# jltsiren/bwt-merge

Measured on AMD Instinct MI355X. Metric: merged Gbases/sec (input1+input2), bit-exact native BWT; value = inputs and result resident in HBM, host_to_host_value = SURVEY 8(d)'s T (page-locked host to page-locked host), higher is better.
Workload: dtype u64

## Files before the change

bwt-merge_amd/__init__.py:

```python
from . import build as _build
from . import capi
from .capi import (Builder, BwtmError, Context, Group, HostBuffer, Index, Locator, Part, host_index, partition_cuts_host, window_blocks, RankArray, Slice, device_bytes_peak, fold_offsets, merged_records, slice_bounds, slice_bounds_equal, init, interleave,
                   make_default_current, merge, merge_consume, merge_host, merge_host_pipelined, merge_host_streamed, assemble_pieces, upload_begin, RESULT_ON_DEVICE, pool_stats, pool_poison_stats, profile_enable, profile_only, profile_read, profile_reset,
                   ra_buffer_bytes, synchronize, trim, tune)



def build(force=False, verbose=False, experimental=False):
    return _build.build(force=force, verbose=verbose, experimental=experimental)
```

bwt-merge_amd/capi.py:

```python
import ctypes as C
import os

import numpy as np

HERE = os.path.dirname(os.path.abspath(__file__))
LIB_PATH = os.environ.get("BWTM_LIB") or os.path.join(HERE, "libbwtm.so")
SIGMA = 6

u64 = C.c_uint64
p_u8 = C.POINTER(C.c_uint8)
p_u64 = C.POINTER(C.c_uint64)
vp = C.c_void_p



class HostInput(C.Structure):
    _fields_ = [("data", C.c_void_p), ("nbytes", u64), ("sequences", u64), ("bases", u64), ("C", p_u64)]


class HostOutput(C.Structure):
    _fields_ = [("data", C.c_void_p), ("nbytes", u64), ("blocks", u64), ("sequences", u64), ("bases", u64),
                ("C", u64 * (SIGMA + 1)), ("block_end", C.c_void_p), ("cum", C.c_void_p),
                ("sample_width", C.c_int), ("fields", C.c_void_p), ("anchors", C.c_void_p),
                ("ms_upload", C.c_double), ("ms_search", C.c_double), ("ms_interleave", C.c_double),
# ... 1148 lines not shown
        except Exception:
            pass


class PoolInfo(C.Structure):
    _fields_ = [("held_bytes", u64), ("cached_bytes", u64), ("peak_bytes", u64), ("mapped_blocks", u64), ("address_bytes_reserved", u64),
                ("address_space_exhausted", C.c_int), ("hipmalloc_fallbacks", u64)]


def pool_stats():
    info = PoolInfo()
    check(lib().bwtm_pool_stats(C.byref(info)))
    return {k: int(getattr(info, k)) for k, _ in PoolInfo._fields_}


def pool_poison_stats():
    fills, nbytes = u64(0), u64(0)
    check(lib().bwtm_pool_poison_stats(C.byref(fills), C.byref(nbytes)))
    return int(fills.value), int(nbytes.value)


def profile_enable(on=True):
    check(lib().bwtm_profile_enable(1 if on else 0))


def profile_only(name=None):
    check(lib().bwtm_profile_only(name.encode() if name else None))


def profile_reset():
    check(lib().bwtm_profile_reset())


def profile_read():
    cap = 64
    names = (C.c_char_p * cap)()
    ms = (C.c_double * cap)()
    n = (u64 * cap)()
    k = lib().bwtm_profile_read(names, ms, n, cap)
    return {names[i].decode(): (ms[i], int(n[i])) for i in range(min(k, cap))}
```

bwt-merge_amd/csrc/api/context.hip.h:

```cpp
#pragma once


namespace
{

thread_local std::string g_error;

int fail(int code, const char* fmt, ...)
{
  char buf[512];
  va_list ap; va_start(ap, fmt); vsnprintf(buf, sizeof(buf), fmt, ap); va_end(ap);
  g_error = buf;
  return code;
}

inline u64 div_up(u64 a, u64 b) { return (a + b - 1) / b; }

}


struct bwtm_context
{
  int device = -1;
  hipStream_t stream = nullptr;
  hipStream_t copy_stream = nullptr;
  std::recursive_mutex mu;
  bool is_default = false;
  std::atomic<long long> live_handles{0};

  bool profiling = false;
  std::string profile_only;
  bool profile_open = false;
  struct Pending { const char* name; hipEvent_t start, stop; };
  std::vector<Pending> pending;
  std::map<std::string, std::pair<double, uint64_t>> totals;
  std::vector<const char*> order;

  std::multimap<u64, void*> free_blocks;
  u64 cached_bytes = 0, held_bytes = 0, peak_bytes = 0;
  struct VBlock { u64 bytes = 0; std::vector<hipMemGenericAllocationHandle_t> chunks; hipEvent_t released = nullptr; };
  bool vmm = false;
  std::vector<hipMemGenericAllocationHandle_t> free_chunks;
  std::map<void*, VBlock> vblocks;
  u64 device_total = 0;
  u64 va_fallbacks = 0;

  void* stream_stage[4] = {nullptr, nullptr, nullptr, nullptr};
  u64 stream_stage_cap[4] = {0, 0, 0, 0};
  u64* host_scratch = nullptr;
  u64 scan1_tiles = 0, pull_scan1_tiles = 0;
};

namespace
{

struct Tuning
{
  long long search_algo = 0;
  long long frontier_unfused = 0;
  long long l1_cap = 0;
  long long emit_path = 0;
  long long round_emits = 1ll << 33;
  long long emit_budget = 0;
  long long frontier_epoch = 512;
  long long eager_cum_budget = 16ll << 30;
  long long upload_chunk = 256ll << 20;
  long long download_chunk = 128ll << 20;
  long long range_ratio = 8;
#ifdef BWTM_EXPERIMENTAL
  long long search_view = 0;
#endif
  long long frontier_stage_out = 1;
  long long frontier_parts = 0;
  long long part_capacity = 0;
  long long recs_uniform = 0;
  long long recs_window = 0;
  long long stream_samples_query = 0;
  long long stream_upload = 0;
  long long extract_batch = 1ll << 20;
  long long locate_batch = 1ll << 20;
  long long overlap_batch = 1ll << 20;
  long long ingest_verify = 0;
#ifdef BWTM_DIAGNOSTICS
  long long walk_emit = 0;
  long long walk_blocks = 0;
  long long walk_kernel = 0;
  long long walk_ablate = 0;
  long long walk_variant = 0;
  long long scatter_kernel = 0;
  long long overlap_kernel = 0;
#endif
};
Tuning g_tune;

std::mutex g_registry_mu;
std::map<int, bwtm_context*> g_default_ctx;
thread_local bwtm_context* t_bound = nullptr;
thread_local bwtm_context* t_ctx = nullptr;

#define CTX (*t_ctx)

#define HIP_TRY(expr) do { hipError_t e_ = (expr); if(e_ != hipSuccess) { \
  return fail(e_ == hipErrorOutOfMemory ? BWTM_ENOMEM : BWTM_ENODEV, "%s failed: %s (%s:%d)", #expr, hipGetErrorString(e_), __FILE__, __LINE__); } } while(0)

#define TRY(expr) do { int rc_ = (expr); if(rc_ != BWTM_OK) { return rc_; } } while(0)
// ... 111 lines not shown
{
  if(!CTX.profile_open) { return; }
  (void)hipEventRecord(CTX.pending.back().stop, CTX.stream);
}

void profile_collect()
{
  if(CTX.pending.empty()) { return; }
  (void)hipStreamSynchronize(CTX.stream);
  for(auto& p : CTX.pending)
  {
    float ms = 0; (void)hipEventElapsedTime(&ms, p.start, p.stop);
    auto it = CTX.totals.find(p.name);
    if(it == CTX.totals.end()) { CTX.totals[p.name] = std::make_pair((double)ms, (uint64_t)1); CTX.order.push_back(p.name); }
    else { it->second.first += ms; it->second.second += 1; }
    (void)hipEventDestroy(p.start); (void)hipEventDestroy(p.stop);
  }
  CTX.pending.clear();
}

#define LAUNCH_CFG(name, kernel, gridx, gridy, block, lds, ...) do { \
  const unsigned long long gx_ = (unsigned long long)(gridx); \
  if(gx_ * (unsigned long long)(block) >= (1ull << 32)) { return fail(BWTM_EINVAL, "launch of %s: %llu workgroups of %u threads do not fit one grid", name, gx_, (unsigned)(block)); } \
  profile_begin(name); \
  hipLaunchKernelGGL(kernel, dim3((unsigned)gx_, (unsigned)(gridy)), dim3((unsigned)(block)), (unsigned)(lds), CTX.stream, __VA_ARGS__); \
  profile_end(); \
  hipError_t le_ = hipGetLastError(); \
  if(le_ != hipSuccess) { return fail(BWTM_ENODEV, "launch of %s failed: %s", name, hipGetErrorString(le_)); } } while(0)

#define LAUNCH(name, kernel, grid, block, ...) LAUNCH_CFG(name, kernel, grid, 1, block, 0, __VA_ARGS__)
#define LAUNCH_LDS(name, kernel, grid, block, lds, ...) LAUNCH_CFG(name, kernel, grid, 1, block, lds, __VA_ARGS__)
#define LAUNCH2D(name, kernel, gridx, gridy, block, ...) LAUNCH_CFG(name, kernel, gridx, gridy, block, 0, __VA_ARGS__)
#define LAUNCH_STEP(name, EMIT, HI, VIEW, PULL, grid, ...) do { \
  if(g_tune.frontier_stage_out) { LAUNCH(name, (k_frontier_step<EMIT, HI, VIEW, PULL, true>), grid, FR_BLOCK, __VA_ARGS__); } \
  else { LAUNCH(name, (k_frontier_step<EMIT, HI, VIEW, PULL, false>), grid, FR_BLOCK, __VA_ARGS__); } } while(0)


u64 VMM_CHUNK = 1024ull << 20;
u64 VMM_MIN = 512ull << 20;

u64 pool_round(u64 n)
{
  if(n < 256) { n = 256; }
  u64 g = (n >= (64ull << 20) ? (2ull << 20) : (n >= (1ull << 20) ? (64ull << 10) : 256ull));
  return (n + g - 1) / g * g;
}

bool trace_enabled()
{
  static const bool on = (std::getenv("BWTM_TRACE") != nullptr);
  return on;
}

double trace_now()
{
  return std::chrono::duration<double, std::milli>(std::chrono::steady_clock::now().time_since_epoch()).count();
}

struct AddressSpace
{
  std::mutex mu;
  char* segment = nullptr; u64 segment_size = 0, used = 0;
  u64 reserved_total = 0;
  bool exhausted = false;
};
AddressSpace g_va;
u64 VA_SEGMENT = 8ull << 40, VA_LIMIT = 64ull << 40;

// ... 296 lines not shown

extern "C" void bwtm_context_destroy(bwtm_context* context)
{
  if(!context || context->is_default) { return; }
  if(t_bound == context) { t_bound = nullptr; }
  if(context->live_handles.load() > 0)
  {
    fail(BWTM_EINVAL, "bwtm_context_destroy: %lld handles of the context are still alive; context not destroyed", context->live_handles.load());
    return;
  }
  context_teardown(context);
  delete context;
}

extern "C" const char* bwtm_last_error(void) { return g_error.c_str(); }

namespace
{
int tune_set(const char* key, long long value)
{
  std::string k(key);
  if(k == "search_algo") { g_tune.search_algo = value; }
  else if(k == "frontier_unfused") { g_tune.frontier_unfused = value; }
  else if(k == "l1_cap") { g_tune.l1_cap = value; }
  else if(k == "emit_path") { g_tune.emit_path = value; }
  else if(k == "round_emits") { g_tune.round_emits = (value > 0 ? value : 1); }
  else if(k == "emit_budget") { g_tune.emit_budget = (value > 0 ? value : 0); }
  else if(k == "frontier_epoch") { g_tune.frontier_epoch = (value > 0 ? value : 512); }
  else if(k == "range_ratio") { g_tune.range_ratio = (value >= 0 ? value : 8); }
#ifdef BWTM_EXPERIMENTAL
  else if(k == "search_view") { g_tune.search_view = (value >= 0 && value <= 2 ? value : 0); }
#endif
  else if(k == "frontier_stage_out") { g_tune.frontier_stage_out = (value != 0); }
  else if(k == "frontier_parts") { g_tune.frontier_parts = (value > 0 ? value : 0); }
  else if(k == "stream_samples_query") { g_tune.stream_samples_query = (value != 0); }
  else if(k == "stream_upload") { g_tune.stream_upload = (value != 0); }
  else if(k == "ingest_verify") { g_tune.ingest_verify = (value != 0); }
  else if(k == "extract_batch") { g_tune.extract_batch = (value > 0 ? value : (1ll << 20)); }
  else if(k == "locate_batch") { g_tune.locate_batch = (value > 0 ? std::min<long long>(value, 1ll << 28) : (1ll << 20)); }
  else if(k == "overlap_batch") { g_tune.overlap_batch = (value > 0 ? std::min<long long>(value, 1ll << 28) : (1ll << 20)); }
  else if(k == "part_capacity") { g_tune.part_capacity = value; }
  else if(k == "recs_uniform") { g_tune.recs_uniform = (value > 0 ? 1 : (value < 0 ? -1 : 0)); }
  else if(k == "recs_window") { g_tune.recs_window = (value == 8192 || value == 16384 || value == 32768 ? value : 0); }
  else if(k == "eager_cum_budget") { g_tune.eager_cum_budget = (value > 0 ? value : (16ll << 30)); }
  else if(k == "upload_chunk") { g_tune.upload_chunk = (value > 0 ? value : (256ll << 20)); }
  else if(k == "download_chunk") { g_tune.download_chunk = (value > 0 ? value : (128ll << 20)); }
#ifdef BWTM_DIAGNOSTICS
  else if(k == "walk_emit") { g_tune.walk_emit = value; }
  else if(k == "walk_blocks") { g_tune.walk_blocks = value; }
  else if(k == "walk_kernel") { g_tune.walk_kernel = value; }
  else if(k == "walk_ablate") { g_tune.walk_ablate = value; }
  else if(k == "walk_variant") { g_tune.walk_variant = value; }
  else if(k == "scatter_kernel") { g_tune.scatter_kernel = value; }
  else if(k == "overlap_kernel") { g_tune.overlap_kernel = (value == 1 ? 1 : 0); }
#endif
  else { return fail(BWTM_EINVAL, "bwtm_tune: unknown key %s", key); }
  return BWTM_OK;
}

void apply_env_tuning()
{
  static std::mutex mu;
  static bool done = false;
  std::lock_guard<std::mutex> lock(mu);
  if(done) { return; }
  done = true;
// ... 73 lines not shown
  if(!out) { return fail(BWTM_EINVAL, "bwtm_host_alloc: null argument"); }
  hipError_t e = hipHostMalloc(out, nbytes > 0 ? nbytes : 8, hipHostMallocDefault);
  if(e != hipSuccess) { (void)hipGetLastError(); return fail(BWTM_ENOMEM, "hipHostMalloc(%llu bytes) failed: %s", (unsigned long long)nbytes, hipGetErrorString(e)); }
  return BWTM_OK;
}

extern "C" void bwtm_host_free(void* p)
{
  if(p) { (void)hipHostFree(p); }
}


extern "C" int bwtm_profile_enable(int on)
{
  ENTER(nullptr);
  profile_collect();
  CTX.profiling = (on != 0);
  return BWTM_OK;
}

extern "C" int bwtm_profile_only(const char* name)
{
  ENTER(nullptr);
  profile_collect();
  CTX.profile_only = (name && name[0] ? std::string(",") + name + "," : std::string());
  return BWTM_OK;
}

extern "C" int bwtm_profile_reset(void)
{
  ENTER(nullptr);
  profile_collect();
  CTX.totals.clear(); CTX.order.clear();
  return BWTM_OK;
}

extern "C" int bwtm_profile_read(const char** names, double* total_ms, uint64_t* launches, int capacity)
{
  Scope scope_(nullptr);
  if(scope_.rc != BWTM_OK) { return 0; }
  profile_collect();
  int k = 0;
  for(const char* name : CTX.order)
  {
    if(k < capacity)
    {
      auto& t = CTX.totals[name];
      names[k] = name; total_ms[k] = t.first; launches[k] = t.second;
    }
    k++;
  }
  return k;
}
```

bwt-merge_amd/csrc/api/search.hip.h:

```cpp
#pragma once

struct bwtm_ra
{
  bwtm_context* ctx = nullptr;
  bwtm_ra() : ctx(t_ctx) { if(ctx) { ctx->live_handles++; } }
  ~bwtm_ra() { if(ctx) { ctx->live_handles--; } }
  bwtm_ra(const bwtm_ra&) = delete; bwtm_ra& operator=(const bwtm_ra&) = delete;
  u64 na = 0, nb = 0, n_out = 0;
  u64 nrecs_out = 0, nchunks = 0;
  DevBuf owned_bits;
  void* bits_ptr = nullptr;
  template<class T> T* bits_as() const { return (T*)bits_ptr; }
  DevBuf chunk_base;
  bool finalized = false;
  u64 values = 0;
  bool ranged = false;
  u64 range_first = 0, range_last = 0;
  DevBuf range_rel;
  DevBuf super_boff;
  bool windowed = false;
  u64 win_word_first = 0, win_words = 0;
};

#define WHOLE_RA(ra, who) if((ra)->windowed) { return fail(BWTM_EINVAL, who ": a window of a rank array (bwtm_ra_create_range) only serves the merge over partitioned records and the output-range entry points"); }
// ... 260 lines not shown
  {
    const u64 limit = std::max<u64>(1, std::min<u64>(count / (u64)g_tune.range_ratio, 1ull << 24));
    TRY(range_phase(a, b, seq_first, count, ra, limit, levels));
    if(levels.N == 0) { return BWTM_OK; }
    TRY(range_alive(levels, node_offsets));
    count = levels.alive;
    if(count == 0) { return BWTM_OK; }
  }
  const u64 ntiles = div_up(ra->n_out + 1, 1ull << TILE_SHIFT);
  const u64 nb_max = div_up(count, FR_BLOCK);
  const u64 nseg = 5 * nb_max;
  const u64 fcap = nb_max * FR_BLOCK;

  const u64 per_seq = b->n / (b->m > 0 ? b->m : 1) + 1;
  u64 emit_budget = (u64)g_tune.emit_budget;
  if(emit_budget == 0)
  {
    emit_budget = 16ull << 30;
    size_t free_b = 0, total_b = 0;
    if(hipMemGetInfo(&free_b, &total_b) == hipSuccess) { emit_budget = std::min<u64>(std::max<u64>(emit_budget, ((u64)free_b + CTX.cached_bytes) / 2), 64ull << 30); }
    else { (void)hipGetLastError(); }
  }
  u64 emit_cap = emit_budget / sizeof(unsigned short);
  if(emit_cap > b->n + 64) { emit_cap = b->n + 64; }
  if(emit_cap > 2 * count * per_seq + (1ull << 20)) { emit_cap = 2 * count * per_seq + (1ull << 20); }
  if(emit_cap < count) { emit_cap = count; }
  u64 EPOCH = std::max<u64>(1, (u64)g_tune.frontier_epoch);
  if(g_tune.l1_cap > 0) { emit_cap = (u64)g_tune.l1_cap; }
  else { EPOCH = std::max<u64>(1, std::min<u64>(EPOCH, emit_cap / std::max<u64>(count, 1))); }
  const u64 bound_budget = 2ull << 30;
  if(EPOCH * (ntiles + 1) * sizeof(u32) > bound_budget) { EPOCH = std::max<u64>(1, bound_budget / ((ntiles + 1) * sizeof(u32))); }

  const bool wide = (a->n >= (1ull << 32) || b->n >= (1ull << 32));
  DevBuf lo[2], hi[2], seg_len[2], seg_phys[2], seg_prefix, emit16, emit_base, bound;
  for(int k = 0; k < 2; k++)
  {
    TRY(lo[k].alloc(fcap * 8)); if(wide) { TRY(hi[k].alloc(fcap * 2)); }
    TRY(seg_len[k].alloc((nseg + 1) * sizeof(u64), true)); TRY(seg_phys[k].alloc((nseg + 1) * sizeof(u64), true));
  }
  TRY(seg_prefix.alloc((nseg + 1) * sizeof(u64)));
  DevBuf first_seg; TRY(first_seg.alloc((nb_max + 1) * sizeof(u32)));
  const u32 LOOK = (count >= (1ull << 24) ? 4 : (count >= (1ull << 20) ? 8 : 32));
  struct Events
  {
    hipEvent_t ev[32]; u32 n = 0;
    ~Events() { for(u32 k = 0; k < n; k++) { (void)hipEventDestroy(ev[k]); } }
  } events;
  for(u32 k = 0; k < LOOK; k++) { HIP_TRY(hipEventCreateWithFlags(&events.ev[k], hipEventDisableTiming)); events.n = k + 1; }
  const u64 scan_tiles = div_up(nseg + 1, (u64)SCAN_TILE);
  DevBuf scan_partial; TRY(scan_partial.alloc(scan_tiles * sizeof(u64), true));
  TRY(emit16.alloc((emit_cap + 16) * sizeof(unsigned short)));
  TRY(emit_base.alloc((EPOCH + 1) * sizeof(u64), true));
  TRY(bound.alloc(EPOCH * (ntiles + 1) * sizeof(u32)));
  HIP_TRY(hipMemsetAsync(bound.p, 0xFF, EPOCH * (ntiles + 1) * sizeof(u32), CTX.stream));

  if(node_phase)
  {
    TRY(range_expand(levels, node_offsets, lo[0].as<uint2>(), hi[0].as<unsigned short>()));
    LAUNCH("frontier_init", k_frontier_init_tables, div_up(nseg + 1, BLOCK_THREADS), BLOCK_THREADS, seg_len[0].as<u64>(), seg_phys[0].as<u64>(), nb_max, count);
    levels.release(); node_offsets.release();
  }
  else
  {
    u64 init_items = (fcap > nseg + 1 ? fcap : nseg + 1);
    LAUNCH("frontier_init", k_frontier_init, div_up(init_items, BLOCK_THREADS), BLOCK_THREADS, lo[0].as<uint2>(), hi[0].as<unsigned short>(),
      seg_len[0].as<u64>(), seg_phys[0].as<u64>(), nb_max, seq_first, count, a->m);
  }
  int cur = 0;
  u64 in_epoch = 0;
  u64 alive_bound = count, epoch_used = 0;
// ... 38 lines not shown
      if(scan_tiles > 1)
      {
        LAUNCH("scan_reduce", k_scan_reduce<0>, scan_tiles, BLOCK_THREADS, seg_len[cur].as<const u64>(), scan_partial.as<u64>(), nseg + 1, (u64)0, scan_tiles);
      }
      LAUNCH("frontier_scan", k_frontier_scan, scan_tiles, BLOCK_THREADS, seg_len[cur].as<const u64>(), scan_partial.as<const u64>(), nseg,
        seg_prefix.as<u64>(), first_seg.as<u32>(), emit_base.as<u64>(), in_epoch, host_ring + (t % LOOK));
      size_in_ring = true;
    }
    else
    {
      TRY(device_scan<0>(seg_len[cur].as<u64>(), seg_prefix.as<u64>(), nseg + 1));
      LAUNCH("frontier_prep", k_frontier_prep, div_up(nseg, BLOCK_THREADS), BLOCK_THREADS, seg_prefix.as<const u64>(), nseg, first_seg.as<u32>(),
        emit_base.as<u64>(), in_epoch);
    }
    if(!size_in_ring) { TRY(fetch_u64(seg_prefix.as<u64>() + nseg, 64 + (u32)(t % LOOK))); HIP_TRY(hipEventRecord(events.ev[t % LOOK], CTX.stream)); }
    {
      const u64 need = std::max<u64>(1, div_up(alive_bound, FR_BLOCK));
      if(g_tune.frontier_parts <= 1 && need * 4 < grid * 3) { grid = need; }
      const int nxt = 1 - cur;
      if(written[nxt] > grid)
      {
        for(u64 c = 0; c < 5; c++) { HIP_TRY(hipMemsetAsync(seg_len[nxt].as<u64>() + c * nb_max + grid, 0, (written[nxt] - grid) * sizeof(u64), CTX.stream)); }
      }
      written[nxt] = grid;
    }
    FrontierView f;
    f.lo = lo[cur].as<const uint2>(); f.hi = hi[cur].as<const unsigned short>();
    f.lo_next = lo[1 - cur].as<uint2>(); f.hi_next = hi[1 - cur].as<unsigned short>();
    f.seg_prefix = seg_prefix.as<const u64>(); f.seg_phys = seg_phys[cur].as<const u64>(); f.first_seg = first_seg.as<const u32>();
    f.seg_len_next = seg_len[1 - cur].as<u64>(); f.seg_phys_next = seg_phys[1 - cur].as<u64>();
    f.nb_max = nb_max;
    f.emit16 = emit16.as<unsigned short>(); f.emit_base = emit_base.as<const u64>(); f.emit_cap = emit_cap; f.bits32 = ra->bits_as<u32>();
    f.bound_row = bound.as<u32>() + in_epoch * (ntiles + 1); f.step = in_epoch; f.block_base = 0; f.src_lo = nullptr; f.src_hi = nullptr; f.nseg_in = 0;
#ifdef BWTM_DIAGNOSTICS
    if(g_tune.walk_emit == 1 && wide) { LAUNCH_STEP("frontier_step_noemit", 1, true, false, false, grid, a->view(), b->view(), f); }
    else if(g_tune.walk_emit == 1) { LAUNCH_STEP("frontier_step_noemit", 1, false, false, false, grid, a->view(), b->view(), f); }
    else
#endif
    if(g_tune.frontier_parts > 1)
    {
      const u64 parts = (u64)g_tune.frontier_parts, per = div_up(nb_max, parts);
      for(u64 part = 0; part < parts && part * per < nb_max; part++)
      {
        f.block_base = (u32)(part * per);
        const u64 nb_part = std::min<u64>(per, nb_max - part * per);
        const char* label = (part == 0 ? "frontier_step_slice0" : "frontier_step_slices");
        if(wide) { LAUNCH_STEP(label, 0, true, false, false, nb_part, a->view(), b->view(), f); }
        else { LAUNCH_STEP(label, 0, false, false, false, nb_part, a->view(), b->view(), f); }
      }
    }
#ifdef BWTM_EXPERIMENTAL
    else if(use_view && wide) { LAUNCH_STEP("frontier_step", 0, true, true, false, grid, a->view(), b->view(), f); }
    else if(use_view) { LAUNCH_STEP("frontier_step", 0, false, true, false, grid, a->view(), b->view(), f); }
#endif
    else if(wide) { LAUNCH_STEP("frontier_step", 0, true, false, false, grid, a->view(), b->view(), f); }
    else { LAUNCH_STEP("frontier_step", 0, false, false, false, grid, a->view(), b->view(), f); }
    if(size_in_ring) { HIP_TRY(hipEventRecord(events.ev[t % LOOK], CTX.stream)); }
    cur = 1 - cur;
    in_epoch++; epoch_used += alive_bound;
    if(in_epoch == EPOCH || (g_tune.l1_cap == 0 && epoch_used + alive_bound > emit_cap))
    {
      TRY(frontier_flush(ra, emit16, emit_cap, emit_base, bound, ntiles, in_epoch));
      HIP_TRY(hipMemsetAsync(bound.p, 0xFF, EPOCH * (ntiles + 1) * sizeof(u32), CTX.stream));
      HIP_TRY(hipMemsetAsync(emit_base.p, 0, (EPOCH + 1) * sizeof(u64), CTX.stream));
      in_epoch = 0; epoch_used = 0;
    }
  }
  TRY(frontier_flush(ra, emit16, emit_cap, emit_base, bound, ntiles, in_epoch));
  return BWTM_OK;
}

}


extern "C" uint64_t bwtm_ra_buffer_bytes(const bwtm_index* a, const bwtm_index* b)
{
  if(!a || !b) { return 0; }
  return div_up(num_records(a->n + b->n), 64) * CHUNK_WORDS * sizeof(u64);
}

extern "C" int bwtm_ra_create_on(const bwtm_index* a, const bwtm_index* b, void* device_buffer, uint64_t nbytes, bwtm_ra** out)
{
  if(!a || !b || !out) { return fail(BWTM_EINVAL, "bwtm_ra_create: null argument"); }
  if(a->ctx != b->ctx) { return fail(BWTM_EINVAL, "bwtm_ra_create: the two indexes live in different contexts"); }
  ENTER(a->ctx);
  bwtm_ra* ra = new bwtm_ra();
  ra->ctx = t_ctx;
  ra->na = a->n; ra->nb = b->n; ra->n_out = a->n + b->n;
  ra->nrecs_out = num_records(ra->n_out);
// ... 168 lines not shown
```

bwt-merge_amd/csrc/kernels/search_frontier.hip.h:

```cpp
#pragma once


constexpr int FR_BLOCK = 256;
constexpr u32 PULL_SRC_SHIFT_ = 56;
constexpr u64 PULL_PHYS_MASK_ = (1ull << PULL_SRC_SHIFT_) - 1;
constexpr int FR_SEGS = 31;

struct FrontierView
{
  const uint2* lo; const unsigned short* hi;
  uint2* lo_next; unsigned short* hi_next;
  const u64* seg_prefix;
  const u64* seg_phys;
  const u32* first_seg;
  u64* seg_len_next; u64* seg_phys_next;
  u64 nb_max;
  unsigned short* emit16;
  const u64* emit_base;
  u64 emit_cap;
  u32* bits32;
  u32* bound_row;
  u64 step;
  u32 block_base;
  const uint2* const* src_lo; const unsigned short* const* src_hi;
// ... 33 lines not shown
__device__ inline void record_words(const RecordFetch& rf, u32 w[16])
{
#pragma unroll
  for(int k = 0; k < 4; k++) { w[4 * k] = rf.v[k].x; w[4 * k + 1] = rf.v[k].y; w[4 * k + 2] = rf.v[k].z; w[4 * k + 3] = rf.v[k].w; }
}

__device__ inline u64 ordinary_lf(const IndexView& X, u64 pos, u32& c, bool want_symbol)
{
  const uint4* p = X.recs + 4 * (pos >> REC_SHIFT);
  const u32 j = (u32)(pos & (REC_POS - 1));
  if(want_symbol)
  {
    const uint4 ch = p[j >> 5];
    const u32 t = j & 31;
    c = ((ch.x >> t) & 1u) | (((ch.y >> t) & 1u) << 1) | (((ch.z >> t) & 1u) << 2);
  }
  if(c == 0) { return 0; }
  u32 total = 0; u32 h[4];
#pragma unroll
  for(u32 k = 0; k < 4; k++)
  {
    const uint4 ch = p[k];
    total += (u32)__builtin_popcount(plane_match(ch.x, ch.y, ch.z, c) & below_mask(j, k));
    h[k] = ch.w;
  }
  const u32 sh = FIELD_BITS * (c - 1);
  const u64 lo = (u64)h[0] | ((u64)h[1] << 32), hi = (u64)h[2] | ((u64)h[3] << 32);
  u64 v;
  if(sh < 64) { v = lo >> sh; if(sh + FIELD_BITS > 64) { v |= hi << (64 - sh); } }
  else { v = hi >> (sh - 64); }
  return X.sup[(pos >> SUPER_SHIFT) * SUP_STRIDE + c] + ((u32)v & FIELD_MASK) + total;
}

template<int EMIT, bool HI, bool VIEW = false, bool PULL = false, bool STAGE = false>
__global__ void __launch_bounds__(FR_BLOCK, (VIEW ? 6 : 8)) k_frontier_step(IndexView A, IndexView B, FrontierView f)
{
  __shared__ u32 wave_cnt[FR_BLOCK / WAVE][6];
  __shared__ uint2 s_out[STAGE ? FR_BLOCK : 1];
  __shared__ unsigned short s_out_hi[STAGE && HI ? FR_BLOCK : 1];
  __shared__ u64 s_prefix[FR_SEGS + 1], s_phys[FR_SEGS + 1];
  __shared__ const uint2* s_src_lo[PULL ? 16 : 1];
  __shared__ const unsigned short* s_src_hi[PULL ? 16 : 1];
  const u64 nseg_out = 5 * f.nb_max;
  const u64 nseg = (PULL ? f.nseg_in : nseg_out);
  const u64 N = f.seg_prefix[nseg];
  const u32 bid = blockIdx.x + f.block_base;
  const u64 g0 = (u64)bid * FR_BLOCK;
  const u32 lane = lane_id(), wave = threadIdx.x >> 6;

  if(g0 >= N)
  {
    if(threadIdx.x < 5) { f.seg_len_next[(u64)threadIdx.x * f.nb_max + bid] = 0; f.seg_phys_next[(u64)threadIdx.x * f.nb_max + bid] = g0; }
    if(bid == 0 && threadIdx.x == 5) { f.seg_len_next[nseg_out] = 0; }
    return;
  }
  const u64 first_seg = f.first_seg[bid];
  if(threadIdx.x <= FR_SEGS)
  {
    u64 sidx = first_seg + threadIdx.x; if(sidx > nseg) { sidx = nseg; }
    s_prefix[threadIdx.x] = f.seg_prefix[sidx];
    s_phys[threadIdx.x] = f.seg_phys[sidx < nseg ? sidx : nseg - 1];
  }
  if(PULL && threadIdx.x >= 64 && threadIdx.x < 80)
  {
    s_src_lo[threadIdx.x - 64] = f.src_lo[threadIdx.x - 64];
    if(HI) { s_src_hi[threadIdx.x - 64] = f.src_hi[threadIdx.x - 64]; }
  }
  __syncthreads();

  const u64 g = g0 + threadIdx.x;
  const bool active = (g < N);
  u64 i = 0, r = 0;
  if(active)
  {
    u64 phys;
    u32 k = 0;
#pragma unroll
    for(u32 step = 16; step != 0; step >>= 1) { if(s_prefix[k + step] <= g) { k += step; } }
    if(k < (u32)FR_SEGS) { phys = s_phys[k] + (g - s_prefix[k]); }
    else
    {
      u64 lo_s = first_seg + FR_SEGS, hi_s = nseg;
      while(hi_s - lo_s > 1)
      {
        const u64 mid = (lo_s + hi_s) >> 1;
        if(f.seg_prefix[mid] <= g) { lo_s = mid; } else { hi_s = mid; }
      }
      const u64 sgm = lo_s;
      phys = f.seg_phys[sgm] + (g - f.seg_prefix[sgm]);
    }
    const uint2* lo_src = f.lo; const unsigned short* hi_src = f.hi;
    if(PULL)
    {
      const u32 src = (u32)(phys >> PULL_SRC_SHIFT_);
      phys &= PULL_PHYS_MASK_;
      lo_src = s_src_lo[src]; if(HI) { hi_src = s_src_hi[src]; }
    }
    uint2 l; u32 h = 0;
    if(PULL) { l = peer_load(&lo_src[phys]); if(HI) { h = (u32)peer_load(&hi_src[phys]); } }
    else { l = lo_src[phys]; if(HI) { h = (u32)hi_src[phys]; } }
    __builtin_amdgcn_sched_barrier(0);
    i = (u64)l.x | ((u64)(h & 0xFF) << 32);
    r = (u64)l.y | ((u64)(h >> 8) << 32);
  }
  const u64 any_active = __ballot(active);
  u32 tile_first = 0xFFFFFFFFu, tile_last = 0xFFFFFFFFu;
  u32 c = 0;
  u64 ni = 0, nr = 0;
  if(any_active != 0)
  {
    const u32 last_lane = 63 - (u32)__builtin_clzll(any_active);
    const u64 li = shfl_u64(i, (int)last_lane), lr = shfl_u64(r, (int)last_lane);
    if(EMIT == 0)
    {
      const u64 p = i + r;
      const u64 my_tile = p >> TILE_SHIFT;
      const u64 prev_tile = shfl_up_u64(my_tile, 1);
      if(active)
      {
        u64 slot = f.emit_base[f.step] + g;
        if(slot < f.emit_cap) { nt_store(&f.emit16[slot], (unsigned short)(p & TILE_MASK)); }
        else { sink_fallback(f.bits32, p); }
        if(lane != 0 && my_tile != prev_tile) { atomicMin(&f.bound_row[my_tile], (u32)g); }
      }
      tile_first = (u32)my_tile;
      tile_last = (u32)shfl_u64(my_tile, (int)last_lane);
    }
#ifdef BWTM_EXPERIMENTAL
    if(VIEW)
    {
      const u64 pi = (active ? i : li), pr = (active ? r : lr);
      const u64 qb = pi / VIEW_POS, qa = pr / VIEW_POS;
      const u32 jb = (u32)(pi - qb * VIEW_POS), ja = (u32)(pr - qa * VIEW_POS);
      RecordFetch fb = record_issue(B.view, B.nview, qb);
      RecordFetch fa = record_issue(A.view, A.nview, qa);
      const u64 vs_b0 = shfl_u64(qb, 0) >> VIEW_SUPER_SHIFT, vs_a0 = shfl_u64(qa, 0) >> VIEW_SUPER_SHIFT;
// ... 41 lines not shown
        ni += cb; nr += ca;
      }
    }
    else
#endif
    {
      u32 wb[16];
      const u64 rec_b = (active ? i : li) >> REC_SHIFT, rec_a = (active ? r : lr) >> REC_SHIFT;
      RecordFetch fb = record_issue(B.recs, B.nrecs, rec_b);
      RecordFetch fa = record_issue(A.recs, A.nrecs, rec_a);
      const u64 sup_b0 = shfl_u64(i, 0) >> SUPER_SHIFT, sup_a0 = shfl_u64(r, 0) >> SUPER_SHIFT;
      const u64* row_b = B.sup + sup_b0 * SUP_STRIDE;
      const u64* row_a = A.sup + sup_a0 * SUP_STRIDE;
      record_words(fb, wb);
      if(active) { c = rec_symbol(wb, (u32)(i & (REC_POS - 1))); }
      u64 supb = 0, supa = 0;
      if(active && c != 0)
      {
        if((i >> SUPER_SHIFT) == sup_b0) { supb = (c == 1 ? row_b[1] : (c == 2 ? row_b[2] : (c == 3 ? row_b[3] : (c == 4 ? row_b[4] : row_b[5])))); }
        else { supb = B.sup[(i >> SUPER_SHIFT) * SUP_STRIDE + c]; }
        if((r >> SUPER_SHIFT) == sup_a0) { supa = (c == 1 ? row_a[1] : (c == 2 ? row_a[2] : (c == 3 ? row_a[3] : (c == 4 ? row_a[4] : row_a[5])))); }
        else { supa = A.sup[(r >> SUPER_SHIFT) * SUP_STRIDE + c]; }
        ni = rec_header(wb, c) + rec_count(wb, c, (u32)(i & (REC_POS - 1)));
      }
      u32 wa[16];
      record_words(fa, wa);
      if(active)
      {
        const u32 ja = (u32)(r & (REC_POS - 1));
        if(c != 0)
        {
          ni += supb;
          nr = supa + rec_header(wa, c) + rec_count(wa, c, ja);
          u64 cb = (c == 1 ? B.C[1] : (c == 2 ? B.C[2] : (c == 3 ? B.C[3] : (c == 4 ? B.C[4] : B.C[5]))));
          u64 ca = (c == 1 ? A.C[1] : (c == 2 ? A.C[2] : (c == 3 ? A.C[3] : (c == 4 ? A.C[4] : A.C[5]))));
          ni += cb; nr += ca;
        }
      }
    }
  }
  u32 my_rank = 0;
  u32 cnt_w[6] = {0, 0, 0, 0, 0, 0};
#pragma unroll
  for(u32 k = 1; k < 6; k++)
  {
    u64 m = __ballot(active && c == k);
    cnt_w[k] = (u32)__builtin_popcountll(m);
    if(c == k) { my_rank = (u32)__builtin_popcountll(m & ((1ull << lane) - 1)); }
  }
  if(lane == 0) { wave_cnt[wave][0] = tile_last; for(u32 k = 1; k < 6; k++) { wave_cnt[wave][k] = cnt_w[k]; } }
  asm volatile("s_waitcnt lgkmcnt(0)" ::: "memory");
  __builtin_amdgcn_s_barrier();
  asm volatile("" ::: "memory");
  const bool mark_first = (EMIT == 0 && lane == 0 && active && (wave == 0 || wave_cnt[wave - 1][0] != tile_first));
  u32 class_base = 0, before_waves = 0;
  u32 tot_k[6] = {0, 0, 0, 0, 0, 0};
#pragma unroll
  for(u32 k = 1; k < 6; k++)
  {
    u32 tot = 0, bw = 0;
    for(u32 w2 = 0; w2 < FR_BLOCK / WAVE; w2++) { u32 v = wave_cnt[w2][k]; if(w2 < wave) { bw += v; } tot += v; }
    if(k < c) { class_base += tot; }
    if(k == c) { before_waves = bw; }
    tot_k[k] = tot;
  }
  if(STAGE)
  {
    if(active && c != 0)
    {
      const u32 at = class_base + before_waves + my_rank;
      s_out[at] = make_uint2((u32)ni, (u32)nr);
      if(HI) { s_out_hi[at] = (unsigned short)(((ni >> 32) & 0xFF) | (((nr >> 32) & 0xFF) << 8)); }
    }
    asm volatile("s_waitcnt lgkmcnt(0)" ::: "memory");
    __builtin_amdgcn_s_barrier();
    asm volatile("" ::: "memory");
    const u32 survivors = tot_k[1] + tot_k[2] + tot_k[3] + tot_k[4] + tot_k[5];
    const uint2 v = s_out[threadIdx.x];
    const unsigned short vh = (HI ? s_out_hi[threadIdx.x] : (unsigned short)0);
    if(threadIdx.x < survivors)
    {
      nt_store(&f.lo_next[g0 + threadIdx.x], v);
      if(HI) { nt_store(&f.hi_next[g0 + threadIdx.x], vh); }
    }
  }
  else if(active && c != 0)
  {
    u64 dst = g0 + class_base + before_waves + my_rank;
    nt_store(&f.lo_next[dst], make_uint2((u32)ni, (u32)nr));
    if(HI) { nt_store(&f.hi_next[dst], (unsigned short)(((ni >> 32) & 0xFF) | (((nr >> 32) & 0xFF) << 8))); }
  }
  if(wave == 0)
  {
    const u32 kk = threadIdx.x + 1;
    u32 tot = 0, base_k = 0;
#pragma unroll
    for(u32 k = 1; k < 6; k++) { if(k == kk) { tot = tot_k[k]; } if(k < kk) { base_k += tot_k[k]; } }
    if(kk < 6)
    {
      f.seg_len_next[(u64)(kk - 1) * f.nb_max + bid] = tot;
      f.seg_phys_next[(u64)(kk - 1) * f.nb_max + bid] = g0 + base_k;
    }
    if(bid == 0 && threadIdx.x == 5) { f.seg_len_next[nseg_out] = 0; }
  }
  if(mark_first) { atomicMin(&f.bound_row[tile_first], (u32)g); }
}

__global__ void __launch_bounds__(BLOCK_THREADS) k_frontier_prep(const u64* seg_prefix, u64 nseg, u32* first_seg, u64* emit_base, u64 step)
{
  u64 sgm = (u64)blockIdx.x * BLOCK_THREADS + threadIdx.x;
  if(sgm == 0) { emit_base[step + 1] = emit_base[step] + seg_prefix[nseg]; }
  if(sgm >= nseg) { return; }
  u64 begin = seg_prefix[sgm], end = seg_prefix[sgm + 1];
  u64 b = (begin + FR_BLOCK - 1) / FR_BLOCK;
  if(b * FR_BLOCK < end) { first_seg[b] = (u32)sgm; }
}

constexpr u64 FRONTIER_SCAN_TILES = 8192;
constexpr u64 FRONTIER_SCAN1_TILES = 1024;

__global__ void __launch_bounds__(BLOCK_THREADS) k_frontier_scan(const u64* seg_len, const u64* partial, u64 nseg, u64* seg_prefix, u32* first_seg,
  u64* emit_base, u64 step, u64* host_n)
{
  __shared__ u64 lds[BLOCK_THREADS / WAVE];
  const u64 n = nseg + 1;
  u64 c = 0;
  for(u64 k = threadIdx.x; k < blockIdx.x; k += BLOCK_THREADS) { c += partial[k]; }
  const u64 carry = block_reduce<0>(c, lds);
  const u64 base = (u64)blockIdx.x * SCAN_TILE + (u64)threadIdx.x * SCAN_ITEMS;
  u64 item[SCAN_ITEMS];
  u64 acc = 0;
#pragma unroll
  for(int k = 0; k < SCAN_ITEMS; k++) { item[k] = seg_len[base + k < n ? base + k : n - 1]; }
#pragma unroll
  for(int k = 0; k < SCAN_ITEMS; k++) { if(base + k >= n) { item[k] = 0; } acc += item[k]; }
  const u64 incl = wave_incl_sum(acc);
  const u64 wave_total = shfl_u64(incl, WAVE - 1);
  u64 excl = shfl_up_u64(incl, 1);
// ... 264 lines not shown
```

include/bwtm.h:

```cpp
#ifndef BWTM_H
#define BWTM_H

#include <stdint.h>

#ifdef __cplusplus
extern "C" {
#endif

#define BWTM_SIGMA 6
#define BWTM_RLE_BLOCK 64

enum
{
  BWTM_OK = 0,
  BWTM_EINVAL = 1,
  BWTM_ENODEV = 2,
  BWTM_ENOMEM = 3,
  BWTM_EALPHABET = 4,
  BWTM_EPEER = 5
};

typedef struct bwtm_context bwtm_context;
typedef struct bwtm_index bwtm_index;
typedef struct bwtm_ra    bwtm_ra;
// ... 218 lines not shown
void bwtm_part_free(bwtm_part* part);
int bwtm_part_window(const bwtm_part* part, int which, uint64_t* pos_first, uint64_t* pos_last);
int bwtm_part_upload(bwtm_part* part, int which, const uint8_t* data, uint64_t nbytes, uint64_t first_position,
                     const uint64_t counts_before[6], int on_device);
int bwtm_part_search(bwtm_part* part);
int bwtm_part_finish(bwtm_part* part, bwtm_slice** slice, uint64_t* byte_offset, uint64_t* total_bytes, uint64_t* next_block_start);
int bwtm_part_stats(const bwtm_part* part, bwtm_part_info* info);


typedef struct bwtm_builder bwtm_builder;

int bwtm_builder_create(uint64_t leaf_reads, bwtm_builder** out);
int bwtm_builder_add(bwtm_builder* builder, const uint8_t* reads, uint64_t nreads, uint32_t width, uint64_t stride,
                     const uint32_t* lengths, int on_device);
uint64_t bwtm_builder_reads(const bwtm_builder* builder);
int bwtm_builder_finish(bwtm_builder* builder, bwtm_index** out);
void bwtm_builder_free(bwtm_builder* builder);

typedef struct
{
  uint64_t held_bytes, cached_bytes, peak_bytes;
  uint64_t mapped_blocks;
  uint64_t address_bytes_reserved;
  int address_space_exhausted;
  uint64_t hipmalloc_fallbacks;
} bwtm_pool_info;
int bwtm_pool_stats(bwtm_pool_info* info);
int bwtm_pool_poison_stats(uint64_t* fills, uint64_t* bytes);


int bwtm_profile_enable(int on);
int bwtm_profile_only(const char* name);
int bwtm_profile_reset(void);
int bwtm_profile_read(const char** names, double* total_ms, uint64_t* launches, int capacity);

#ifdef __cplusplus
}
#endif

#endif
```

Measured before the change: 91.89.

## Store frontier ranks class-relative to drop the high-byte array for wide inputs

For wide inputs where every class fits in 32 bits, the frontier step now writes class-relative ranks without the C[c] offset. That removes the 2-byte hi array writes and reads after the first step. The next step restores the absolute rank by adding C[class], which it picks from the segment index. This saves frontier memory traffic and allocation but adds a per-element class lookup, plus more template instantiations and a launch counter for observability.

```diff
diff --git a/bwt-merge_amd/__init__.py b/bwt-merge_amd/__init__.py
--- a/bwt-merge_amd/__init__.py
+++ b/bwt-merge_amd/__init__.py
@@ -1,7 +1,7 @@
 from . import build as _build
 from . import capi
 from .capi import (Builder, BwtmError, Context, Group, HostBuffer, Index, Locator, Part, host_index, partition_cuts_host, window_blocks, RankArray, Slice, device_bytes_peak, fold_offsets, merged_records, slice_bounds, slice_bounds_equal, init, interleave,
-                   make_default_current, merge, merge_consume, merge_host, merge_host_pipelined, merge_host_streamed, assemble_pieces, upload_begin, RESULT_ON_DEVICE, pool_stats, pool_poison_stats, profile_enable, profile_only, profile_read, profile_reset,
+                   make_default_current, merge, merge_consume, merge_host, merge_host_pipelined, merge_host_streamed, assemble_pieces, upload_begin, RESULT_ON_DEVICE, pool_stats, pool_poison_stats, profile_enable, profile_only, profile_read, profile_reset, frontier_step_forms,
                    ra_buffer_bytes, synchronize, trim, tune)
 
 
diff --git a/bwt-merge_amd/capi.py b/bwt-merge_amd/capi.py
--- a/bwt-merge_amd/capi.py
+++ b/bwt-merge_amd/capi.py
@@ -1204,6 +1204,14 @@
     check(lib().bwtm_profile_reset())
 
 
+def frontier_step_forms():
+    f = lib().bwtm_frontier_step_forms
+    f.restype = C.c_int; f.argtypes = [p_u64]
+    n = (u64 * 3)()
+    check(f(n))
+    return tuple(int(v) for v in n)
+
+
 def profile_read():
     cap = 64
     names = (C.c_char_p * cap)()
diff --git a/bwt-merge_amd/csrc/api/context.hip.h b/bwt-merge_amd/csrc/api/context.hip.h
--- a/bwt-merge_amd/csrc/api/context.hip.h
+++ b/bwt-merge_amd/csrc/api/context.hip.h
@@ -49,6 +49,7 @@
   u64 stream_stage_cap[4] = {0, 0, 0, 0};
   u64* host_scratch = nullptr;
   u64 scan1_tiles = 0, pull_scan1_tiles = 0;
+  u64 step_forms[3] = {0, 0, 0};
 };
 
 namespace
@@ -71,6 +72,7 @@
   long long search_view = 0;
 #endif
   long long frontier_stage_out = 1;
+  long long frontier_rel = 1;
   long long frontier_parts = 0;
   long long part_capacity = 0;
   long long recs_uniform = 0;
@@ -248,8 +250,17 @@
 #define LAUNCH_LDS(name, kernel, grid, block, lds, ...) LAUNCH_CFG(name, kernel, grid, 1, block, lds, __VA_ARGS__)
 #define LAUNCH2D(name, kernel, gridx, gridy, block, ...) LAUNCH_CFG(name, kernel, gridx, gridy, block, 0, __VA_ARGS__)
 #define LAUNCH_STEP(name, EMIT, HI, VIEW, PULL, grid, ...) do { \
+  CTX.step_forms[0]++; \
   if(g_tune.frontier_stage_out) { LAUNCH(name, (k_frontier_step<EMIT, HI, VIEW, PULL, true>), grid, FR_BLOCK, __VA_ARGS__); } \
   else { LAUNCH(name, (k_frontier_step<EMIT, HI, VIEW, PULL, false>), grid, FR_BLOCK, __VA_ARGS__); } } while(0)
+#define LAUNCH_STEP_FORM(name, EMIT, HI, REL, grid, ...) do { \
+  CTX.step_forms[REL]++; \
+  if(g_tune.frontier_stage_out) { LAUNCH(name, (k_frontier_step<Rel<REL>, EMIT, HI, true>), grid, FR_BLOCK, __VA_ARGS__); } \
+  else { LAUNCH(name, (k_frontier_step<Rel<REL>, EMIT, HI, false>), grid, FR_BLOCK, __VA_ARGS__); } } while(0)
+#define LAUNCH_STEP_REL(name, EMIT, HI, rel, grid, ...) do { \
+  if((rel) == 2) { LAUNCH_STEP_FORM(name, EMIT, false, 2, grid, __VA_ARGS__); } \
+  else if((rel) == 1) { LAUNCH_STEP_FORM(name, EMIT, HI, 1, grid, __VA_ARGS__); } \
+  else { LAUNCH_STEP(name, EMIT, HI, false, false, grid, __VA_ARGS__); } } while(0)
 
 
 u64 VMM_CHUNK = 1024ull << 20;
@@ -612,6 +623,7 @@
   else if(k == "search_view") { g_tune.search_view = (value >= 0 && value <= 2 ? value : 0); }
 #endif
   else if(k == "frontier_stage_out") { g_tune.frontier_stage_out = (value != 0); }
+  else if(k == "frontier_rel") { g_tune.frontier_rel = (value >= 0 && value <= 2 ? value : 1); }
   else if(k == "frontier_parts") { g_tune.frontier_parts = (value > 0 ? value : 0); }
   else if(k == "stream_samples_query") { g_tune.stream_samples_query = (value != 0); }
   else if(k == "stream_upload") { g_tune.stream_upload = (value != 0); }
@@ -751,6 +763,15 @@
   ENTER(nullptr);
   profile_collect();
   CTX.totals.clear(); CTX.order.clear();
+  for(int k = 0; k < 3; k++) { CTX.step_forms[k] = 0; }
+  return BWTM_OK;
+}
+
+extern "C" int bwtm_frontier_step_forms(uint64_t launches[3])
+{
+  if(!launches) { return fail(BWTM_EINVAL, "bwtm_frontier_step_forms: null argument"); }
+  ENTER(nullptr);
+  for(int k = 0; k < 3; k++) { launches[k] = CTX.step_forms[k]; }
   return BWTM_OK;
 }
 
diff --git a/bwt-merge_amd/csrc/api/search.hip.h b/bwt-merge_amd/csrc/api/search.hip.h
--- a/bwt-merge_amd/csrc/api/search.hip.h
+++ b/bwt-merge_amd/csrc/api/search.hip.h
@@ -316,10 +316,15 @@
   if(EPOCH * (ntiles + 1) * sizeof(u32) > bound_budget) { EPOCH = std::max<u64>(1, bound_budget / ((ntiles + 1) * sizeof(u32))); }
 
   const bool wide = (a->n >= (1ull << 32) || b->n >= (1ull << 32));
+  bool rel = (g_tune.frontier_rel == 2 || (g_tune.frontier_rel == 1 && wide));
+  for(int c = 1; c <= 5 && rel; c++) { rel = (a->C[c + 1] - a->C[c] < (1ull << 32) && b->C[c + 1] - b->C[c] < (1ull << 32)); }
+#ifdef BWTM_EXPERIMENTAL
+  if(g_tune.search_view != 0) { rel = false; }
+#endif
   DevBuf lo[2], hi[2], seg_len[2], seg_phys[2], seg_prefix, emit16, emit_base, bound;
   for(int k = 0; k < 2; k++)
   {
-    TRY(lo[k].alloc(fcap * 8)); if(wide) { TRY(hi[k].alloc(fcap * 2)); }
+    TRY(lo[k].alloc(fcap * 8)); if(wide && (k == 0 || !rel)) { TRY(hi[k].alloc(fcap * 2)); }
     TRY(seg_len[k].alloc((nseg + 1) * sizeof(u64), true)); TRY(seg_phys[k].alloc((nseg + 1) * sizeof(u64), true));
   }
   TRY(seg_prefix.alloc((nseg + 1) * sizeof(u64)));
@@ -424,9 +429,10 @@
     f.nb_max = nb_max;
     f.emit16 = emit16.as<unsigned short>(); f.emit_base = emit_base.as<const u64>(); f.emit_cap = emit_cap; f.bits32 = ra->bits_as<u32>();
     f.bound_row = bound.as<u32>() + in_epoch * (ntiles + 1); f.step = in_epoch; f.block_base = 0; f.src_lo = nullptr; f.src_hi = nullptr; f.nseg_in = 0;
+    const int rel_form = (rel ? (t == 0 ? 1 : 2) : 0);
 #ifdef BWTM_DIAGNOSTICS
-    if(g_tune.walk_emit == 1 && wide) { LAUNCH_STEP("frontier_step_noemit", 1, true, false, false, grid, a->view(), b->view(), f); }
-    else if(g_tune.walk_emit == 1) { LAUNCH_STEP("frontier_step_noemit", 1, false, false, false, grid, a->view(), b->view(), f); }
+    if(g_tune.walk_emit == 1 && wide) { LAUNCH_STEP_REL("frontier_step_noemit", 1, true, rel_form, grid, a->view(), b->view(), f); }
+    else if(g_tune.walk_emit == 1) { LAUNCH_STEP_REL("frontier_step_noemit", 1, false, rel_form, grid, a->view(), b->view(), f); }
     else
 #endif
     if(g_tune.frontier_parts > 1)
@@ -437,16 +443,17 @@
         f.block_base = (u32)(part * per);
         const u64 nb_part = std::min<u64>(per, nb_max - part * per);
         const char* label = (part == 0 ? "frontier_step_slice0" : "frontier_step_slices");
-        if(wide) { LAUNCH_STEP(label, 0, true, false, false, nb_part, a->view(), b->view(), f); }
-        else { LAUNCH_STEP(label, 0, false, false, false, nb_part, a->view(), b->view(), f); }
+        if(wide) { LAUNCH_STEP_REL(label, 0, true, rel_form, nb_part, a->view(), b->view(), f); }
+        else { LAUNCH_STEP_REL(label, 0, false, rel_form, nb_part, a->view(), b->view(), f); }
       }
     }
 #ifdef BWTM_EXPERIMENTAL
     else if(use_view && wide) { LAUNCH_STEP("frontier_step", 0, true, true, false, grid, a->view(), b->view(), f); }
     else if(use_view) { LAUNCH_STEP("frontier_step", 0, false, true, false, grid, a->view(), b->view(), f); }
 #endif
-    else if(wide) { LAUNCH_STEP("frontier_step", 0, true, false, false, grid, a->view(), b->view(), f); }
-    else { LAUNCH_STEP("frontier_step", 0, false, false, false, grid, a->view(), b->view(), f); }
+    else if(wide) { LAUNCH_STEP_REL("frontier_step", 0, true, rel_form, grid, a->view(), b->view(), f); }
+    else { LAUNCH_STEP_REL("frontier_step", 0, false, rel_form, grid, a->view(), b->view(), f); }
+    if(rel && t == 0) { hi[0].release(); }
     if(size_in_ring) { HIP_TRY(hipEventRecord(events.ev[t % LOOK], CTX.stream)); }
     cur = 1 - cur;
     in_epoch++; epoch_used += alive_bound;
diff --git a/bwt-merge_amd/csrc/kernels/search_frontier.hip.h b/bwt-merge_amd/csrc/kernels/search_frontier.hip.h
--- a/bwt-merge_amd/csrc/kernels/search_frontier.hip.h
+++ b/bwt-merge_amd/csrc/kernels/search_frontier.hip.h
@@ -89,12 +89,14 @@
   return X.sup[(pos >> SUPER_SHIFT) * SUP_STRIDE + c] + ((u32)v & FIELD_MASK) + total;
 }
 
-template<int EMIT, bool HI, bool VIEW = false, bool PULL = false, bool STAGE = false>
-__global__ void __launch_bounds__(FR_BLOCK, (VIEW ? 6 : 8)) k_frontier_step(IndexView A, IndexView B, FrontierView f)
-{
+template<int EMIT, bool HI, bool VIEW, bool PULL, bool STAGE, int REL>
+__device__ __forceinline__ void frontier_step_body(const IndexView A, const IndexView B, const FrontierView f)
+{
+  static_assert(REL >= 0 && REL <= 2 && (REL == 0 || (!VIEW && !PULL)) && (REL != 2 || !HI), "class-relative coordinates: the plain search only");
+  constexpr bool HI_OUT = (HI && REL == 0);
   __shared__ u32 wave_cnt[FR_BLOCK / WAVE][6];
   __shared__ uint2 s_out[STAGE ? FR_BLOCK : 1];
-  __shared__ unsigned short s_out_hi[STAGE && HI ? FR_BLOCK : 1];
+  __shared__ unsigned short s_out_hi[STAGE && HI_OUT ? FR_BLOCK : 1];
   __shared__ u64 s_prefix[FR_SEGS + 1], s_phys[FR_SEGS + 1];
   __shared__ const uint2* s_src_lo[PULL ? 16 : 1];
   __shared__ const unsigned short* s_src_hi[PULL ? 16 : 1];
@@ -130,11 +132,11 @@
   u64 i = 0, r = 0;
   if(active)
   {
-    u64 phys;
+    u64 phys, seg;
     u32 k = 0;
 #pragma unroll
     for(u32 step = 16; step != 0; step >>= 1) { if(s_prefix[k + step] <= g) { k += step; } }
-    if(k < (u32)FR_SEGS) { phys = s_phys[k] + (g - s_prefix[k]); }
+    if(k < (u32)FR_SEGS) { seg = first_seg + k; phys = s_phys[k] + (g - s_prefix[k]); }
     else
     {
       u64 lo_s = first_seg + FR_SEGS, hi_s = nseg;
@@ -144,6 +146,7 @@
         if(f.seg_prefix[mid] <= g) { lo_s = mid; } else { hi_s = mid; }
       }
       const u64 sgm = lo_s;
+      seg = sgm;
       phys = f.seg_phys[sgm] + (g - f.seg_prefix[sgm]);
     }
     const uint2* lo_src = f.lo; const unsigned short* hi_src = f.hi;
@@ -159,6 +162,12 @@
     __builtin_amdgcn_sched_barrier(0);
     i = (u64)l.x | ((u64)(h & 0xFF) << 32);
     r = (u64)l.y | ((u64)(h >> 8) << 32);
+    if(REL == 2)
+    {
+      const u64 nb1 = f.nb_max, nb2 = 2 * f.nb_max, nb3 = 3 * f.nb_max, nb4 = 4 * f.nb_max;
+      i += (seg < nb1 ? B.C[1] : (seg < nb2 ? B.C[2] : (seg < nb3 ? B.C[3] : (seg < nb4 ? B.C[4] : B.C[5]))));
+      r += (seg < nb1 ? A.C[1] : (seg < nb2 ? A.C[2] : (seg < nb3 ? A.C[3] : (seg < nb4 ? A.C[4] : A.C[5]))));
+    }
   }
   const u64 any_active = __ballot(active);
   u32 tile_first = 0xFFFFFFFFu, tile_last = 0xFFFFFFFFu;
@@ -266,9 +275,12 @@
         {
           ni += supb;
           nr = supa + rec_header(wa, c) + rec_count(wa, c, ja);
-          u64 cb = (c == 1 ? B.C[1] : (c == 2 ? B.C[2] : (c == 3 ? B.C[3] : (c == 4 ? B.C[4] : B.C[5]))));
-          u64 ca = (c == 1 ? A.C[1] : (c == 2 ? A.C[2] : (c == 3 ? A.C[3] : (c == 4 ? A.C[4] : A.C[5]))));
-          ni += cb; nr += ca;
+          if(REL == 0)
+          {
+            u64 cb = (c == 1 ? B.C[1] : (c == 2 ? B.C[2] : (c == 3 ? B.C[3] : (c == 4 ? B.C[4] : B.C[5]))));
+            u64 ca = (c == 1 ? A.C[1] : (c == 2 ? A.C[2] : (c == 3 ? A.C[3] : (c == 4 ? A.C[4] : A.C[5]))));
+            ni += cb; nr += ca;
+          }
         }
       }
     }
@@ -304,25 +316,25 @@
     {
       const u32 at = class_base + before_waves + my_rank;
       s_out[at] = make_uint2((u32)ni, (u32)nr);
-      if(HI) { s_out_hi[at] = (unsigned short)(((ni >> 32) & 0xFF) | (((nr >> 32) & 0xFF) << 8)); }
+      if(HI_OUT) { s_out_hi[at] = (unsigned short)(((ni >> 32) & 0xFF) | (((nr >> 32) & 0xFF) << 8)); }
     }
     asm volatile("s_waitcnt lgkmcnt(0)" ::: "memory");
     __builtin_amdgcn_s_barrier();
     asm volatile("" ::: "memory");
     const u32 survivors = tot_k[1] + tot_k[2] + tot_k[3] + tot_k[4] + tot_k[5];
     const uint2 v = s_out[threadIdx.x];
-    const unsigned short vh = (HI ? s_out_hi[threadIdx.x] : (unsigned short)0);
+    const unsigned short vh = (HI_OUT ? s_out_hi[threadIdx.x] : (unsigned short)0);
     if(threadIdx.x < survivors)
     {
       nt_store(&f.lo_next[g0 + threadIdx.x], v);
-      if(HI) { nt_store(&f.hi_next[g0 + threadIdx.x], vh); }
+      if(HI_OUT) { nt_store(&f.hi_next[g0 + threadIdx.x], vh); }
     }
   }
   else if(active && c != 0)
   {
     u64 dst = g0 + class_base + before_waves + my_rank;
     nt_store(&f.lo_next[dst], make_uint2((u32)ni, (u32)nr));
-    if(HI) { nt_store(&f.hi_next[dst], (unsigned short)(((ni >> 32) & 0xFF) | (((nr >> 32) & 0xFF) << 8))); }
+    if(HI_OUT) { nt_store(&f.hi_next[dst], (unsigned short)(((ni >> 32) & 0xFF) | (((nr >> 32) & 0xFF) << 8))); }
   }
   if(wave == 0)
   {
@@ -338,6 +350,19 @@
     if(bid == 0 && threadIdx.x == 5) { f.seg_len_next[nseg_out] = 0; }
   }
   if(mark_first) { atomicMin(&f.bound_row[tile_first], (u32)g); }
+}
+
+template<int EMIT, bool HI, bool VIEW = false, bool PULL = false, bool STAGE = false>
+__global__ void __launch_bounds__(FR_BLOCK, (VIEW ? 6 : 8)) k_frontier_step(IndexView A, IndexView B, FrontierView f)
+{
+  frontier_step_body<EMIT, HI, VIEW, PULL, STAGE, 0>(A, B, f);
+}
+
+template<int REL> struct Rel { static constexpr int value = REL; };
+template<class FORM, int EMIT, bool HI, bool STAGE>
+__global__ void __launch_bounds__(FR_BLOCK, 8) k_frontier_step(IndexView A, IndexView B, FrontierView f)
+{
+  frontier_step_body<EMIT, HI, false, false, STAGE, FORM::value>(A, B, f);
 }
 
 __global__ void __launch_bounds__(BLOCK_THREADS) k_frontier_prep(const u64* seg_prefix, u64 nseg, u32* first_seg, u64* emit_base, u64 step)
diff --git a/include/bwtm.h b/include/bwtm.h
--- a/include/bwtm.h
+++ b/include/bwtm.h
@@ -274,6 +274,7 @@
 int bwtm_profile_enable(int on);
 int bwtm_profile_only(const char* name);
 int bwtm_profile_reset(void);
+int bwtm_frontier_step_forms(uint64_t launches[3]);
 int bwtm_profile_read(const char** names, double* total_ms, uint64_t* launches, int capacity);
 
 #ifdef __cplusplus
```

After: 94.57 (median of 6 runs). +2.9%, better.
